# clementabary/music2dance

Hardware: AMD Instinct MI355X
Metric: 120-frame seq/sec, phase3 WGAN-GP step, batch 64 per GPU (higher is better)
Workload: dtype f32

## Files before the change

music2dance_amd/csrc/conv1d_thin.hip:

```cpp
#include "m2d_common.h"

#define THIN_MAX_K 32

struct ThinArgs {
  const float* x;
  const float* w;
  const float* bias;
  const float* dy;
  const float* mask;
  float* out;
  float* out2;
  float* stats;
  int xT, xS, xhop;
  int B, L, Cout, ks, stride, pad, Lout;
  int act;
  float slope, mask_slope;
  int chunk;
};

typedef float thin_f32x16 __attribute__((ext_vector_type(16)));
typedef float thin_f32x4 __attribute__((ext_vector_type(4)));
typedef unsigned thin_u32x4 __attribute__((ext_vector_type(4)));

__device__ __forceinline__ float thin_act(float v, int act, float slope) {
  if (act == 0) return v;
  if (act == 1) return m2d_act_sel(v, 1, 0.f);
  return m2d_act_sel(v, 2, slope);
}

template <int KS, int S, bool MASKED>
__global__ void __launch_bounds__(256) thin_bwd_weight_mfma_kernel(const ThinArgs a) {
  constexpr int LD = 65;
  constexpr int XW = 64 * S + 32;
  constexpr int DEPTH = MASKED ? 1 : 2;
  __shared__ float smem[4][32 * LD + XW];
  const int lane = threadIdx.x & 63, wave = threadIdx.x >> 6;
  const int n = blockIdx.y;
  const int l0 = blockIdx.x * a.chunk;
  int l1 = l0 + a.chunk;
  if (l1 > a.Lout) l1 = a.Lout;
  const float* xr = a.xT > 0 ? a.x + (size_t)(n / a.xT) * a.xS + (size_t)(n % a.xT) * a.xhop : a.x + (size_t)n * a.L;
  const float* dyn = a.dy + (size_t)n * 32 * a.Lout;
  const float* mkn = (MASKED && a.mask) ? a.mask + (size_t)n * 32 * a.Lout : nullptr;
  float* tl = smem[wave];
  float* xw = tl + 32 * LD;
  thin_f32x16 acc;
#pragma unroll
  for (int r = 0; r < 16; ++r) acc[r] = 0.f;
  const int i31 = lane & 31, h = lane >> 5;
  const int lq = 4 * (lane & 15);
  const bool vec = (a.Lout % 4) == 0, vec2 = (a.Lout % 2) == 0 && (l0 & 1) == 0;
  float4 dv[DEPTH][8], mv[MASKED ? 8 : 1];
  float xs[DEPTH][(XW + 63) / 64];
  auto fetch = [&](float4 (&d4)[8], float (&xq)[(XW + 63) / 64], int lt) {
#ifdef THIN_X_BW_NOLOAD
#pragma unroll
    for (int i = 0; i < 8; ++i) {
      d4[i] = make_float4((float)lt, 1.f, 2.f, (float)lane);
      if (MASKED) mv[i] = make_float4(1.f, -1.f, 1.f, (float)(lane - 32));
    }
#pragma unroll
    for (int i = 0; i < (XW + 63) / 64; ++i) xq[i] = (float)(lt + i);
    return;
#endif
#pragma unroll
    for (int i = 0; i < 8; ++i) {
      const int co = (lane >> 4) + 4 * i;
      const size_t g = (size_t)co * a.Lout + lt + lq;
      if (vec && lt + lq + 3 < l1) {
        d4[i] = *reinterpret_cast<const float4*>(dyn + g);
        if (MASKED) mv[i] = mkn ? *reinterpret_cast<const float4*>(mkn + g) : make_float4(1.f, 1.f, 1.f, 1.f);
      } else if (vec2 && lt + lq + 3 < l1) {
        const float2 d0 = *reinterpret_cast<const float2*>(dyn + g);
        const float2 d1 = *reinterpret_cast<const float2*>(dyn + g + 2);
        d4[i] = make_float4(d0.x, d0.y, d1.x, d1.y);
        if (MASKED) {
          if (mkn) {
            const float2 m0 = *reinterpret_cast<const float2*>(mkn + g);
            const float2 m1 = *reinterpret_cast<const float2*>(mkn + g + 2);
            mv[i] = make_float4(m0.x, m0.y, m1.x, m1.y);
          } else {
            mv[i] = make_float4(1.f, 1.f, 1.f, 1.f);
          }
        }
      } else {
        float d[4], m[4];
#pragma unroll
        for (int j = 0; j < 4; ++j) {
          const bool ok = lt + lq + j < l1;
          d[j] = ok ? dyn[g + j] : 0.f;
          m[j] = (MASKED && ok && mkn) ? mkn[g + j] : 1.f;
        }
        d4[i] = make_float4(d[0], d[1], d[2], d[3]);
        if (MASKED) mv[i] = make_float4(m[0], m[1], m[2], m[3]);
      }
    }
#pragma unroll
    for (int i = 0; i < (XW + 63) / 64; ++i) {
      const int e = lane + 64 * i;
      const int pos = lt * S - a.pad + e;
      xq[i] = (e < XW && lt < l1 && pos >= 0 && pos < a.L) ? xr[pos] : 0.f;
    }
  };
  const int lt0 = l0 + wave * 64;
#pragma unroll
  for (int d = 0; d < DEPTH; ++d)
    if (lt0 + 256 * d < l1) fetch(dv[d], xs[d], lt0 + 256 * d);
  for (int lt = lt0; lt < l1; lt += 256) {
#pragma unroll
    for (int i = 0; i < 8; ++i) {
      const int co = (lane >> 4) + 4 * i;
      const float ms = a.mask_slope;
      tl[co * LD + lq + 0] = dv[0][i].x * ((!MASKED || mv[i].x > 0.f) ? 1.f : ms);
      tl[co * LD + lq + 1] = dv[0][i].y * ((!MASKED || mv[i].y > 0.f) ? 1.f : ms);
      tl[co * LD + lq + 2] = dv[0][i].z * ((!MASKED || mv[i].z > 0.f) ? 1.f : ms);
      tl[co * LD + lq + 3] = dv[0][i].w * ((!MASKED || mv[i].w > 0.f) ? 1.f : ms);
    }
#pragma unroll
    for (int i = 0; i < (XW + 63) / 64; ++i)
      if (lane + 64 * i < XW) xw[lane + 64 * i] = xs[0][i];
    __builtin_amdgcn_fence(__ATOMIC_RELEASE, "wavefront");
    __builtin_amdgcn_wave_barrier();
    if (DEPTH == 2) {
#pragma unroll
      for (int i = 0; i < 8; ++i) dv[0][i] = dv[DEPTH - 1][i];
#pragma unroll
      for (int i = 0; i < (XW + 63) / 64; ++i) xs[0][i] = xs[DEPTH - 1][i];
    }
    if (lt + 256 * DEPTH < l1) fetch(dv[DEPTH - 1], xs[DEPTH - 1], lt + 256 * DEPTH);
    const float* xa = xw + S * h + i31;
    const float* bb = tl + i31 * LD + h;
#pragma unroll 8
    for (int j = 0; j < 32; ++j) {
      float av = xa[2 * S * j];
      if (KS < 32) av = i31 == 31 ? 1.f : av;
#ifdef THIN_X_BW_NOMFMA
      acc[j & 15] += av * bb[2 * j];
#else
      acc = __builtin_amdgcn_mfma_f32_32x32x2f32(av, bb[2 * j], acc, 0, 0, 0);
#endif
    }
    __builtin_amdgcn_wave_barrier();
  }
  __syncthreads();
  float* red = &smem[0][0];
#pragma unroll
  for (int r = 0; r < 16; ++r) red[wave * 1024 + ((r & 3) + 8 * (r >> 2) + 4 * h) * 32 + i31] = acc[r];
  __syncthreads();
  const size_t blk = (size_t)blockIdx.y * gridDim.x + blockIdx.x;
  for (int o = threadIdx.x; o < 32 * KS; o += 256) {
    const int co = o / KS, kk = o % KS;
    const int idx = kk * 32 + co;
    a.out[blk * 32 * KS + o] = red[idx] + red[1024 + idx] + red[2048 + idx] + red[3072 + idx];
  }
  if (a.out2 && threadIdx.x < 32) {
    const int idx = 31 * 32 + threadIdx.x;
    a.out2[blk * 32 + threadIdx.x] = red[idx] + red[1024 + idx] + red[2048 + idx] + red[3072 + idx];
  }
}

template <int KS, int S, bool MASKED>
__global__ void __launch_bounds__(256) thin_bwd_data_mfma_kernel(const ThinArgs a) {
  constexpr int LD = 65;
  constexpr int ZLD = 33;
  constexpr int T = (KS + S - 1) / S;
  constexpr int HALO = T - 1;
  constexpr int DEPTH = MASKED ? 1 : 2;
  __shared__ float smem[4][(64 + HALO) * ZLD];
  static_assert((64 + HALO) * ZLD >= 32 * LD, "image size");
  const int lane = threadIdx.x & 63, wave = threadIdx.x >> 6;
  const int l31 = lane & 31, h = lane >> 5;
  const int n = blockIdx.y;
  const int nq = (a.L - 1 + a.pad) / S + 1;
  const int run = a.chunk / 4;
  const int qa = blockIdx.x * a.chunk + wave * run;
  int qb = qa + run;
  if (qb > nq) qb = nq;
  if (qa >= nq) return;
  const float* dyn = a.dy + (size_t)n * 32 * a.Lout;
  const float* mkn = (MASKED && a.mask) ? a.mask + (size_t)n * 32 * a.Lout : nullptr;
  float* dxn = a.out + (size_t)n * a.L;
  float* buf = smem[wave];
  float wa[16];
#pragma unroll
  for (int s2 = 0; s2 < 16; ++s2) wa[s2] = l31 < KS ? a.w[(2 * s2 + h) * KS + l31] : 0.f;
  const int lq = 4 * (lane & 15);
  const bool vec = (a.Lout % 4) == 0, vec2 = (a.Lout % 2) == 0;
  float4 dv[DEPTH][8], mv[MASKED ? 8 : 1];
  auto fetch = [&](float4 (&d4)[8], int lt) {
#pragma unroll
    for (int i = 0; i < 8; ++i) {
      const int co = (lane >> 4) + 4 * i;
      const int l = lt + lq;
      const size_t g = (size_t)co * a.Lout + l;
      if (vec && l >= 0 && l + 3 < a.Lout) {
        d4[i] = *reinterpret_cast<const float4*>(dyn + g);
        if (MASKED) mv[i] = mkn ? *reinterpret_cast<const float4*>(mkn + g) : make_float4(1.f, 1.f, 1.f, 1.f);
      } else if (vec2 && l >= 0 && l + 3 < a.Lout) {
        const float2 d0 = *reinterpret_cast<const float2*>(dyn + g);
        const float2 d1 = *reinterpret_cast<const float2*>(dyn + g + 2);
        d4[i] = make_float4(d0.x, d0.y, d1.x, d1.y);
        if (MASKED) {
          if (mkn) {
            const float2 m0 = *reinterpret_cast<const float2*>(mkn + g);
            const float2 m1 = *reinterpret_cast<const float2*>(mkn + g + 2);
            mv[i] = make_float4(m0.x, m0.y, m1.x, m1.y);
          } else {
            mv[i] = make_float4(1.f, 1.f, 1.f, 1.f);
          }
        }
      } else {
        float d[4], m[4];
#pragma unroll
        for (int j = 0; j < 4; ++j) {
          const bool ok = l + j >= 0 && l + j < a.Lout;
          d[j] = ok ? dyn[(ptrdiff_t)g + j] : 0.f;
          m[j] = (MASKED && ok && mkn) ? mkn[(ptrdiff_t)g + j] : 1.f;
        }
        d4[i] = make_float4(d[0], d[1], d[2], d[3]);
        if (MASKED) mv[i] = make_float4(m[0], m[1], m[2], m[3]);
      }
    }
  };
  auto land = [&](const float4 (&d4)[8]) {
#pragma unroll
    for (int i = 0; i < 8; ++i) {
      const int co = (lane >> 4) + 4 * i;
      const float ms = a.mask_slope;
      buf[co * LD + lq + 0] = d4[i].x * ((!MASKED || mv[i].x > 0.f) ? 1.f : ms);
      buf[co * LD + lq + 1] = d4[i].y * ((!MASKED || mv[i].y > 0.f) ? 1.f : ms);
      buf[co * LD + lq + 2] = d4[i].z * ((!MASKED || mv[i].z > 0.f) ? 1.f : ms);
      buf[co * LD + lq + 3] = d4[i].w * ((!MASKED || mv[i].w > 0.f) ? 1.f : ms);
    }
  };
  auto sync = [&]() {
    __builtin_amdgcn_fence(__ATOMIC_RELEASE, "wavefront");
    __builtin_amdgcn_wave_barrier();
    __builtin_amdgcn_fence(__ATOMIC_ACQUIRE, "wavefront");
  };
  auto zmma = [&](int c0) {
    thin_f32x16 acc;
#pragma unroll
    for (int r = 0; r < 16; ++r) acc[r] = 0.f;
#pragma unroll
    for (int s2 = 0; s2 < 16; ++s2)
      acc = __builtin_amdgcn_mfma_f32_32x32x2f32(wa[s2], buf[(2 * s2 + h) * LD + c0 + l31], acc, 0, 0, 0);
    return acc;
  };
  float carry[3] = {0.f, 0.f, 0.f};
  if (qa > 0) {
    fetch(dv[0], qa - 64);
    land(dv[0]);
    sync();
    const thin_f32x16 z = zmma(32);
    sync();
#pragma unroll
    for (int r = 0; r < 16; ++r)
      if (l31 >= 32 - HALO) buf[(l31 - (32 - HALO)) * ZLD + (r & 3) + 8 * (r >> 2) + 4 * h] = z[r];
    sync();
#pragma unroll
    for (int k = 0; k < 3; ++k) carry[k] = buf[((lane + 64 * k) >> 5) * ZLD + ((lane + 64 * k) & 31)];
    sync();
  }
#pragma unroll
  for (int d = 0; d < DEPTH; ++d)
    if (qa + 64 * d < qb) fetch(dv[d], qa + 64 * d);
  for (int l0 = qa; l0 < qb; l0 += 64) {
    land(dv[0]);
    sync();
    if (DEPTH == 2) {
#pragma unroll
      for (int i = 0; i < 8; ++i) dv[0][i] = dv[1][i];
    }
    if (l0 + 64 * DEPTH < qb) fetch(dv[DEPTH - 1], l0 + 64 * DEPTH);
    const thin_f32x16 z0 = zmma(0), z1 = zmma(32);
    sync();
#pragma unroll
    for (int k = 0; k < 3; ++k) buf[((lane + 64 * k) >> 5) * ZLD + ((lane + 64 * k) & 31)] = carry[k];
#pragma unroll
    for (int r = 0; r < 16; ++r) {
      const int kk = (r & 3) + 8 * (r >> 2) + 4 * h;
      buf[(HALO + l31) * ZLD + kk] = z0[r];
      buf[(HALO + 32 + l31) * ZLD + kk] = z1[r];
    }
    sync();
    float o[S];
#pragma unroll
    for (int rho = 0; rho < S; ++rho) {
      float acc = 0.f;
#pragma unroll
      for (int t = 0; t < T; ++t)
        if (rho + S * t < KS) acc += buf[(HALO + lane - t) * ZLD + rho + S * t];
      o[rho] = acc;
    }
#pragma unroll
    for (int k = 0; k < 3; ++k) carry[k] = buf[(64 + ((lane + 64 * k) >> 5)) * ZLD + ((lane + 64 * k) & 31)];
    sync();
#pragma unroll
    for (int rho = 0; rho < S; ++rho) buf[S * lane + rho] = o[rho];
    sync();
    const int j0 = S * l0 - a.pad;
#pragma unroll
    for (int k = 0; k < S; ++k) {
      const int e = lane + 64 * k;
      const int j = j0 + e;
      if (j >= 0 && j < a.L && l0 + e / S < qb) dxn[j] = buf[e];
    }
    sync();
  }
}

__global__ void __launch_bounds__(256) thin_sum_partials_kernel(const float* partial, float* dw, int nblk, int n_out,
                                                                  const float* partial2, float* out2, int n_out2) {
  __shared__ double part[32][8];
  const int ox = threadIdx.x & 7, g = threadIdx.x >> 3;
  const int nb1 = (n_out + 7) / 8;
  int blk = blockIdx.x;
  if (blk >= nb1) {
    blk -= nb1;
    partial = partial2;
    dw = out2;
    n_out = n_out2;
  }
  const int o = blk * 8 + ox;
  double s = 0.0;
  if (o < n_out)
    for (int b = g; b < nblk; b += 32) s += (double)partial[(size_t)b * n_out + o];
  part[g][ox] = s;
  __syncthreads();
  if (g == 0 && o < n_out) {
    double t = 0.0;
#pragma unroll
    for (int j = 0; j < 32; ++j) t += part[j][ox];
    dw[o] = (float)t;
  }
}

static bool thin_ok(int Cin, int Cout, int ks, int stride) {
  return Cin == 1 && ks == 25 && stride == 4 && Cout == 32;
}

bool m2d_thin_applicable(int Cin, int Cout, int ks, int stride) { return thin_ok(Cin, Cout, ks, stride); }

static int thin_bw_chunk(int B, int Lout) {
  const long long per = ((long long)B * Lout + 511) / 512;
  long long c = (per + 255) / 256 * 256;
  if (c < 1024) c = 1024;
  if (c > 8192) c = 8192;
  return (int)c;
}

size_t m2d_thin_bwd_weight_ws(int B, int Cout, int ks, int Lout) {
  const size_t nblk = (size_t)B * m2d_ceil_div(Lout, thin_bw_chunk(B, Lout));
  return nblk * (Cout * ks + Cout) * sizeof(float);
}

template <int KS, int S>
#ifndef THIN_WPE
#define THIN_WPE 4
#endif
__global__ void __launch_bounds__(256) __attribute__((amdgpu_waves_per_eu(THIN_WPE, 8)))
thin_fwd_mfma_kernel(const ThinArgs a, int tiles_per_row, int total_tiles) {
  constexpr int NS = (KS + 1) / 2;
  constexpr int LDP = 32 + 4;
  __shared__ float img[4][32 * LDP];
  const int lane = threadIdx.x & 63, wave = __builtin_amdgcn_readfirstlane(threadIdx.x >> 6);
  const int c31 = lane & 31, h = lane >> 5;
  float* im = img[wave];
  float wa[NS];
#pragma unroll
  for (int ks = 0; ks < NS; ++ks) {
    const int k = 2 * ks + h;
    wa[ks] = k < KS ? a.w[c31 * KS + k] : 0.f;
  }
  const int nwaves = gridDim.x * 4;
  const int valign = (a.Lout % 4 == 0) ? 4 : (a.Lout % 2 == 0) ? 2 : 1;
  const int cq = lane & 7;
  const int crow = lane >> 3;
  float bv[4];
#pragma unroll
  for (int i = 0; i < 4; ++i) bv[i] = a.bias ? a.bias[crow + 8 * i] : 0.f;
  const float ms = a.mask_slope;
  double st1[4] = {0.0, 0.0, 0.0, 0.0}, st2[4] = {0.0, 0.0, 0.0, 0.0};
  const unsigned row_bytes = (unsigned)a.Lout * 4u;
  const unsigned sample_bytes = 32u * row_bytes;
  constexpr bool LAST_DEAD = (KS & 1) != 0;

  auto fetch = [&](int tile, float (&dst)[NS]) {
    const int n = tile / tiles_per_row;
    const int p0 = (tile - n * tiles_per_row) * 32;
    const float* xr = a.xT > 0 ? a.x + (size_t)(n / a.xT) * a.xS + (size_t)(n % a.xT) * a.xhop : a.x + (size_t)n * a.L;
    const __amdgpu_buffer_rsrc_t rx = __builtin_amdgcn_make_buffer_rsrc((void*)xr, (short)0, (int)((unsigned)a.L * 4u), 0x00020000);
    const int l = p0 + c31;
    const unsigned voff = l < a.Lout ? (unsigned)((l * S - a.pad + h) * 4) : 0x80000000u;
#pragma unroll
    for (int ks = 0; ks < NS; ++ks) {
#ifdef THIN_X_NOGATHER
      dst[ks] = (float)((voff + ks) & 7);
#else
      dst[ks] = __builtin_bit_cast(float, __builtin_amdgcn_raw_buffer_load_b32(rx, (int)voff + 8 * ks, 0, 0));
#endif
    }
    if (LAST_DEAD && h == 1) dst[NS - 1] = 0.f;
  };
  auto process = [&](int tile, const float (&xb)[NS]) {
    const int n = tile / tiles_per_row;
    const int p0 = (tile - n * tiles_per_row) * 32;
    const bool interior = valign == 4 && p0 + 32 <= a.Lout;
    const __amdgpu_buffer_rsrc_t ro = __builtin_amdgcn_make_buffer_rsrc((void*)(a.out + (size_t)n * 32 * a.Lout), (short)0, (int)sample_bytes, 0x00020000);
    const __amdgpu_buffer_rsrc_t rm = __builtin_amdgcn_make_buffer_rsrc((void*)((a.mask ? a.mask : a.out) + (size_t)n * 32 * a.Lout), (short)0,
                                                                        (int)(a.mask ? sample_bytes : 0u), 0x00020000);
    const unsigned eo = (unsigned)crow * row_bytes + (unsigned)(p0 + 4 * cq) * 4u;
    thin_f32x4 mk[4];
    if (interior && a.mask) {
#pragma unroll
      for (int i = 0; i < 4; ++i)
        mk[i] = __builtin_bit_cast(thin_f32x4, __builtin_amdgcn_raw_buffer_load_b128(rm, (int)(eo + (unsigned)(8 * i) * row_bytes), 0, 0));
    }
    thin_f32x16 acc;
#pragma unroll
    for (int r = 0; r < 16; ++r) acc[r] = 0.f;
#pragma unroll
    for (int ks = 0; ks < NS; ++ks) acc = __builtin_amdgcn_mfma_f32_32x32x2f32(wa[ks], xb[ks], acc, 0, 0, 0);
#pragma unroll
    for (int r = 0; r < 16; ++r) im[((r & 3) + 8 * (r >> 2) + 4 * h) * LDP + c31] = acc[r];
    __builtin_amdgcn_fence(__ATOMIC_RELEASE, "wavefront");
    __builtin_amdgcn_wave_barrier();
    __builtin_amdgcn_fence(__ATOMIC_ACQUIRE, "wavefront");
    if (interior) {
#pragma unroll
      for (int i = 0; i < 4; ++i) {
        const int co = crow + 8 * i;
        const thin_f32x4 q = *reinterpret_cast<const thin_f32x4*>(im + co * LDP + 4 * cq);
        thin_f32x4 v;
#pragma unroll
        for (int j = 0; j < 4; ++j) v[j] = thin_act(q[j] + bv[i], a.act, a.slope);
        if (a.mask) {
#pragma unroll
          for (int j = 0; j < 4; ++j) v[j] *= mk[i][j] > 0.f ? 1.f : ms;
        }
#ifdef THIN_X_NOSTORE
        if (v[0] == 12345.678f)
#endif
        __builtin_amdgcn_raw_buffer_store_b128(__builtin_bit_cast(thin_u32x4, v), ro, (int)(eo + (unsigned)(8 * i) * row_bytes), 0, 0);
        st1[i] += (v[0] + v[1]) + (v[2] + v[3]);
        st2[i] += (v[0] * v[0] + v[1] * v[1]) + (v[2] * v[2] + v[3] * v[3]);
      }
    } else {
      const bool whole = p0 + 4 * cq + 4 <= a.Lout;
#pragma unroll 1
      for (int i = 0; i < 4; ++i) {
        const int co = crow + 8 * i;
        const float4 q = *reinterpret_cast<const float4*>(im + co * LDP + 4 * cq);
        const float b_ = i == 0 ? bv[0] : (i == 1 ? bv[1] : (i == 2 ? bv[2] : bv[3]));
        float v[4] = {q.x + b_, q.y + b_, q.z + b_, q.w + b_};
        const size_t o = ((size_t)n * 32 + co) * a.Lout + p0 + 4 * cq;
#pragma unroll
        for (int j = 0; j < 4; ++j) v[j] = thin_act(v[j], a.act, a.slope);
        if (whole && valign == 4) {
          if (a.mask) {
            const float4 m = *reinterpret_cast<const float4*>(a.mask + o);
            v[0] *= m.x > 0.f ? 1.f : ms;
            v[1] *= m.y > 0.f ? 1.f : ms;
            v[2] *= m.z > 0.f ? 1.f : ms;
            v[3] *= m.w > 0.f ? 1.f : ms;
          }
          *reinterpret_cast<float4*>(a.out + o) = make_float4(v[0], v[1], v[2], v[3]);
        } else if (whole && valign == 2) {
          if (a.mask) {
            const float2 m0 = *reinterpret_cast<const float2*>(a.mask + o);
            const float2 m1 = *reinterpret_cast<const float2*>(a.mask + o + 2);
            v[0] *= m0.x > 0.f ? 1.f : ms;
            v[1] *= m0.y > 0.f ? 1.f : ms;
            v[2] *= m1.x > 0.f ? 1.f : ms;
            v[3] *= m1.y > 0.f ? 1.f : ms;
          }
          *reinterpret_cast<float2*>(a.out + o) = make_float2(v[0], v[1]);
          *reinterpret_cast<float2*>(a.out + o + 2) = make_float2(v[2], v[3]);
        } else {
#pragma unroll
          for (int j = 0; j < 4; ++j) {
            if (p0 + 4 * cq + j < a.Lout) {
              float y = v[j];
              if (a.mask) y *= a.mask[o + j] > 0.f ? 1.f : ms;
              a.out[o + j] = y;
              v[j] = y;
            } else {
              v[j] = 0.f;
            }
          }
        }
        {
          const float t1 = (v[0] + v[1]) + (v[2] + v[3]);
          const float t2 = (v[0] * v[0] + v[1] * v[1]) + (v[2] * v[2] + v[3] * v[3]);
          if (i == 0) { st1[0] += t1; st2[0] += t2; }
          else if (i == 1) { st1[1] += t1; st2[1] += t2; }
          else if (i == 2) { st1[2] += t1; st2[2] += t2; }
          else { st1[3] += t1; st2[3] += t2; }
        }
      }
    }
    __builtin_amdgcn_wave_barrier();
  };

  int tile = __builtin_amdgcn_readfirstlane(blockIdx.x * 4 + wave);
  const int gw = tile;
  auto flush_stats = [&]() {
    if (!a.stats) return;
#pragma unroll
    for (int i = 0; i < 4; ++i) {
      double s1 = st1[i], s2 = st2[i];
#pragma unroll
      for (int off = 4; off > 0; off >>= 1) {
        s1 += __shfl_xor(s1, off, 64);
        s2 += __shfl_xor(s2, off, 64);
      }
      if (cq == 0) {
        float* dst = a.stats + (size_t)gw * 64 + 2 * (crow + 8 * i);
        dst[0] = (float)s1;
        dst[1] = (float)s2;
      }
    }
  };
  if (tile >= total_tiles) {
    flush_stats();
    return;
  }
  float xa[NS], xb2[NS];
  fetch(tile, xa);
#pragma unroll 1
  for (;;) {
    const int t2 = tile + nwaves;
    if (t2 < total_tiles) fetch(t2, xb2);
    process(tile, xa);
    if (t2 >= total_tiles) break;
    const int t3 = t2 + nwaves;
    if (t3 < total_tiles) fetch(t3, xa);
    process(t2, xb2);
    if (t3 >= total_tiles) break;
    tile = t3;
  }
  flush_stats();
}

struct M2dWinView {
  int T, S, hop;
};

int m2d_rowsums_reduce(const float* part, int P, int M, double* sums, double* scratch, hipStream_t stream);

static int thin_fwd_tiles_per_row(int Lout) { return m2d_ceil_div(Lout, 32); }
#define THIN_FWD_MAX_WAVES (256 * 16 * 4)
static size_t thin_fwd_stats_part(int B, int Lout) { (void)B; (void)Lout; return (size_t)THIN_FWD_MAX_WAVES * 64 * sizeof(float); }
size_t m2d_thin_fwd_stats_ws(int B, int Lout) { return thin_fwd_stats_part(B, Lout) + (size_t)256 * 32 * 2 * sizeof(double); }
static int thin_fwd_grid(int total_tiles) {
  static const int per_cu = [] { const char* e = getenv("M2D_THIN_WG_PER_CU"); const int v = e ? atoi(e) : THIN_WPE; return v >= 1 && v <= 16 ? v : THIN_WPE; }();
  const int need = m2d_ceil_div(total_tiles, 4), full = 256 * per_cu;
  return need < full ? need : full;
}

int m2d_thin_fwd(const float* x, const float* w, const float* bias, float* y, int B, int L, int Cout, int ks,
                 int stride, int pad, int Lout, int act, float slope, const float* out_mask, float out_mask_slope,
                 const M2dWinView* wv, double* stats, void* ws, size_t ws_bytes, hipStream_t stream) {
  ThinArgs a;
  memset(&a, 0, sizeof(a));
  if (wv) { a.xT = wv->T; a.xS = wv->S; a.xhop = wv->hop; }
  const int tpr = thin_fwd_tiles_per_row(Lout);
  if ((long long)B * tpr >= (1LL << 30) || (long long)Lout * 32 * 4 >= (1LL << 31) || (long long)L * 4 >= (1LL << 31))
    M2D_FAIL(M2D_ERR_RANGE, "m2d_conv1d_fwd (thin): too many tiles / a sample beyond 2 GiB");
  const int total = B * tpr;
  if (stats) {
    if (!ws || ws_bytes < m2d_thin_fwd_stats_ws(B, Lout)) M2D_FAIL(M2D_ERR_WORKSPACE, "m2d_conv1d_fwd (thin): no room for the statistics partials");
    a.stats = (float*)ws;
  }
  a.x = x; a.w = w; a.bias = bias; a.mask = out_mask; a.out = y;
  a.B = B; a.L = L; a.Cout = Cout; a.ks = ks; a.stride = stride; a.pad = pad; a.Lout = Lout;
  a.act = act; a.slope = slope; a.mask_slope = out_mask_slope;
  M2dProfScope prof(M2D_FAM_POINTWISE, stream, 2.0 * B * Lout * (double)Cout * ks,
                    4.0 * B * ((double)L + (double)Cout * Lout * (out_mask ? 2 : 1)), "thin_conv_fwd", Cout, B * Lout, ks);
  const int grid = thin_fwd_grid(total);
  hipLaunchKernelGGL((thin_fwd_mfma_kernel<25, 4>), dim3(grid), dim3(256), 0, stream, a, tpr, total);
  M2D_CHECK_LAUNCH("thin_fwd_mfma_kernel");
  if (stats)
    return m2d_rowsums_reduce(a.stats, grid * 4, 32, stats, (double*)((char*)a.stats + thin_fwd_stats_part(B, Lout)), stream);
  return M2D_OK;
}

template <int KS, int S>
__global__ void __launch_bounds__(512) thin_long_fwd_kernel(const ThinArgs a, int tiles_per_row, int total_tiles) {
  static_assert(KS % 2 == 0 && S % 2 == 0, "even taps / stride");
  constexpr int NS = KS / 2;
  constexpr int SEG = 31 * S + KS + 3;
  constexpr int SEG4 = (SEG + 3) / 4;
  constexpr int NP = (SEG4 + 63) / 64;
  constexpr int LDP = 32 + 4;
  constexpr int WAVE_FLOATS = SEG4 * 4 + 32 * LDP;
  extern __shared__ __attribute__((aligned(16))) float lsm[];
  float* Ws = lsm;
  const int lane = threadIdx.x & 63, wave = __builtin_amdgcn_readfirstlane(threadIdx.x >> 6);
  float* xs = lsm + KS * 32 + wave * WAVE_FLOATS;
  float* im = xs + SEG4 * 4;
  const int c31 = lane & 31, h = lane >> 5;
  const int lead = ((a.pad + 3) & ~3) - a.pad;
  for (int e = threadIdx.x; e < KS * 32; e += 512) {
    const int k = e >> 5, c = e & 31;
    Ws[e] = a.w[c * KS + k];
  }
  __syncthreads();
  const int nwaves = gridDim.x * 8;
  const int cq = lane & 7, crow = lane >> 3;
  float bv[4];
#pragma unroll
  for (int i = 0; i < 4; ++i) bv[i] = a.bias ? a.bias[crow + 8 * i] : 0.f;
  const unsigned row_bytes = (unsigned)a.Lout * 4u;
  const unsigned sample_bytes = 32u * row_bytes;

  thin_f32x4 seg[NP];
  auto fetch = [&](int tile) {
    const int n = tile / tiles_per_row;
    const int p0 = (tile - n * tiles_per_row) * 32;
    const float* xr = a.xT > 0 ? a.x + (size_t)(n / a.xT) * a.xS + (size_t)(n % a.xT) * a.xhop : a.x + (size_t)n * a.L;
    const __amdgpu_buffer_rsrc_t rx = __builtin_amdgcn_make_buffer_rsrc((void*)xr, (short)0, (int)((unsigned)a.L * 4u), 0x00020000);
    const int first = p0 * S - a.pad - lead;
#pragma unroll
    for (int i = 0; i < NP; ++i) {
      const int q = lane + 64 * i;
      const unsigned voff = q < SEG4 ? (unsigned)((first + 4 * q) * 4) : 0x80000000u;
      seg[i] = __builtin_bit_cast(thin_f32x4, __builtin_amdgcn_raw_buffer_load_b128(rx, (int)voff, 0, 0));
    }
  };
  auto land = [&]() {
#pragma unroll
    for (int i = 0; i < NP; ++i) {
      const int q = lane + 64 * i;
      if (q < SEG4) *reinterpret_cast<thin_f32x4*>(xs + 4 * q) = seg[i];
    }
  };
  int tile = __builtin_amdgcn_readfirstlane(blockIdx.x * 8 + wave);
  const int gw = tile;
  double st1[4] = {0.0, 0.0, 0.0, 0.0}, st2[4] = {0.0, 0.0, 0.0, 0.0};
  auto flush_stats = [&]() {
    if (!a.stats) return;
#pragma unroll
    for (int i = 0; i < 4; ++i) {
      double s1 = st1[i], s2 = st2[i];
#pragma unroll
      for (int off = 4; off > 0; off >>= 1) {
        s1 += __shfl_xor(s1, off, 64);
        s2 += __shfl_xor(s2, off, 64);
      }
      if (cq == 0) {
        float* dst = a.stats + (size_t)gw * 64 + 2 * (crow + 8 * i);
        dst[0] = (float)s1;
        dst[1] = (float)s2;
      }
    }
  };
  if (tile >= total_tiles) {
    flush_stats();
    return;
  }
  fetch(tile);
  land();
  __builtin_amdgcn_fence(__ATOMIC_RELEASE, "wavefront");
  __builtin_amdgcn_wave_barrier();
  __builtin_amdgcn_fence(__ATOMIC_ACQUIRE, "wavefront");
  const float* ap = Ws + h * 32 + c31;
  const float* bp = xs + c31 * S + h + lead;
#pragma unroll 1
  for (;;) {
    const int next = tile + nwaves;
    if (next < total_tiles) fetch(next);
    thin_f32x16 acc;
#pragma unroll
    for (int r = 0; r < 16; ++r) acc[r] = 0.f;
#pragma unroll
    for (int ks = 0; ks < NS; ++ks) acc = __builtin_amdgcn_mfma_f32_32x32x2f32(ap[ks * 64], bp[2 * ks], acc, 0, 0, 0);
    const int n = tile / tiles_per_row;
    const int p0 = (tile - n * tiles_per_row) * 32;
#pragma unroll
    for (int r = 0; r < 16; ++r) im[((r & 3) + 8 * (r >> 2) + 4 * h) * LDP + c31] = acc[r];
    __builtin_amdgcn_fence(__ATOMIC_RELEASE, "wavefront");
    __builtin_amdgcn_wave_barrier();
    __builtin_amdgcn_fence(__ATOMIC_ACQUIRE, "wavefront");
    if (next < total_tiles) land();
    const __amdgpu_buffer_rsrc_t ro = __builtin_amdgcn_make_buffer_rsrc((void*)(a.out + (size_t)n * 32 * a.Lout), (short)0, (int)sample_bytes, 0x00020000);
    const unsigned eo = (unsigned)crow * row_bytes + (unsigned)(p0 + 4 * cq) * 4u;
#pragma unroll
    for (int i = 0; i < 4; ++i) {
      const int co = crow + 8 * i;
      const thin_f32x4 q = *reinterpret_cast<const thin_f32x4*>(im + co * LDP + 4 * cq);
      thin_f32x4 v;
#pragma unroll
      for (int j = 0; j < 4; ++j) v[j] = thin_act(q[j] + bv[i], a.act, a.slope);
      __builtin_amdgcn_raw_buffer_store_b128(__builtin_bit_cast(thin_u32x4, v), ro, (int)(eo + (unsigned)(8 * i) * row_bytes), 0, 0);
      st1[i] += (v[0] + v[1]) + (v[2] + v[3]);
      st2[i] += (v[0] * v[0] + v[1] * v[1]) + (v[2] * v[2] + v[3] * v[3]);
    }
    __builtin_amdgcn_fence(__ATOMIC_RELEASE, "wavefront");
    __builtin_amdgcn_wave_barrier();
    __builtin_amdgcn_fence(__ATOMIC_ACQUIRE, "wavefront");
    if (next >= total_tiles) break;
    tile = next;
  }
  flush_stats();
}

static bool thin_long_enabled() {
  static const bool on = [] { const char* e = getenv("M2D_THIN_LONG"); return !(e && e[0] == '0'); }();
  return on;
}
static int thin_long_kind(int Cin, int Cout, int ks, int stride) {
  if (Cin != 1 || Cout != 32) return 0;
  if (ks == 250 && stride == 50) return 1;
  if (ks == 160 && stride == 4) return 2;
  return 0;
}
bool m2d_thin_long_applicable(int Cin, int Cout, int ks, int stride, int pad, int L) {
  if (!thin_long_enabled() || !thin_long_kind(Cin, Cout, ks, stride)) return false;
  if ((L & 3) || pad < 0 || pad >= ks) return false;
  const int Lout = (L + 2 * pad - ks) / stride + 1;
  return Lout > 0 && Lout % 32 == 0;
}
#define THIN_LONG_MAX_WAVES (512 * 8)
size_t m2d_thin_long_stats_ws(int B, int Lout) { (void)B; (void)Lout; return (size_t)THIN_LONG_MAX_WAVES * 64 * sizeof(float) + (size_t)256 * 32 * 2 * sizeof(double); }

template <int KS, int S>
static int thin_long_launch(const ThinArgs& a, int tpr, int total, hipStream_t stream, int* waves) {
  constexpr int SEG4 = (31 * S + KS + 3 + 3) / 4;
  constexpr size_t lds = (size_t)(KS * 32 + 8 * (SEG4 * 4 + 32 * 36)) * sizeof(float);
  static const bool attr_ok = hipFuncSetAttribute(reinterpret_cast<const void*>(&thin_long_fwd_kernel<KS, S>),
                                                  hipFuncAttributeMaxDynamicSharedMemorySize, (int)lds) == hipSuccess;
  if (!attr_ok) M2D_FAIL(M2D_ERR_HIP, "m2d_conv1d_fwd (long single-channel kernel): cannot reserve %zu bytes of LDS", lds);
  const int per_cu = lds * 2 <= 160 * 1024 ? 2 : 1;
  const int need = m2d_ceil_div(total, 8);
  const int grid = need < 256 * per_cu ? need : 256 * per_cu;
  *waves = grid * 8;
  hipLaunchKernelGGL((thin_long_fwd_kernel<KS, S>), dim3(grid), dim3(512), lds, stream, a, tpr, total);
  M2D_CHECK_LAUNCH("thin_long_fwd_kernel");
  return M2D_OK;
}

int m2d_thin_long_fwd(const float* x, const float* w, const float* bias, float* y, int B, int L, int ks, int stride, int pad,
                      int Lout, int act, float slope, const M2dWinView* wv, double* stats, void* ws, size_t ws_bytes,
                      hipStream_t stream) {
  ThinArgs a;
  memset(&a, 0, sizeof(a));
  if (wv) { a.xT = wv->T; a.xS = wv->S; a.xhop = wv->hop; }
  const int tpr = Lout / 32;
  if ((long long)B * tpr >= (1LL << 30) || (long long)Lout * 32 * 4 >= (1LL << 31) || (long long)L * 4 >= (1LL << 31))
    M2D_FAIL(M2D_ERR_RANGE, "m2d_conv1d_fwd (long single-channel kernel): too many tiles / a sample beyond 2 GiB");
  const int total = B * tpr;
  const size_t part = (size_t)THIN_LONG_MAX_WAVES * 64 * sizeof(float);
  if (stats) {
    if (!ws || ws_bytes < m2d_thin_long_stats_ws(B, Lout)) M2D_FAIL(M2D_ERR_WORKSPACE, "m2d_conv1d_fwd (long single-channel kernel): no room for the statistics partials");
    a.stats = (float*)ws;
  }
  a.x = x; a.w = w; a.bias = bias; a.out = y;
  a.B = B; a.L = L; a.Cout = 32; a.ks = ks; a.stride = stride; a.pad = pad; a.Lout = Lout;
  a.act = act; a.slope = slope;
  M2dProfScope prof(M2D_FAM_GEMM, stream, 2.0 * B * Lout * 32.0 * ks, 0.0, "m2d_conv1d_fwd", 32, B * Lout, ks);
  int rc, waves = 0;
  if (thin_long_kind(1, 32, ks, stride) == 1) rc = thin_long_launch<250, 50>(a, tpr, total, stream, &waves);
  else rc = thin_long_launch<160, 4>(a, tpr, total, stream, &waves);
  if (rc) return rc;
  if (stats) return m2d_rowsums_reduce(a.stats, waves, 32, stats, (double*)((char*)a.stats + part), stream);
  return M2D_OK;
}

int m2d_thin_bwd_data(const float* dy, const float* w, float* dx, int B, int L, int Cout, int ks, int stride,
                      int pad, int Lout, const float* dy_mask, float dy_mask_slope, hipStream_t stream) {
  ThinArgs a;
  memset(&a, 0, sizeof(a));
  a.dy = dy; a.w = w; a.mask = dy_mask; a.out = dx;
  a.B = B; a.L = L; a.Cout = Cout; a.ks = ks; a.stride = stride; a.pad = pad; a.Lout = Lout;
  a.mask_slope = dy_mask_slope;
  const int nq = (L - 1 + pad) / stride + 1;
  M2dProfScope prof(M2D_FAM_POINTWISE, stream, 2.0 * B * Lout * (double)Cout * ks,
                    4.0 * B * ((double)L + (double)Cout * Lout * (dy_mask ? 2 : 1)), "thin_conv_bwd_data", 1, B * L, Cout * ks);
  a.chunk = thin_bw_chunk(B, nq);
  const dim3 grid(m2d_ceil_div(nq, a.chunk), B);
  if (dy_mask) hipLaunchKernelGGL((thin_bwd_data_mfma_kernel<25, 4, true>), grid, dim3(256), 0, stream, a);
  else hipLaunchKernelGGL((thin_bwd_data_mfma_kernel<25, 4, false>), grid, dim3(256), 0, stream, a);
  M2D_CHECK_LAUNCH("thin_bwd_data_mfma_kernel");
  return M2D_OK;
}

int m2d_thin_bwd_weight(const float* x, const float* dy, float* dw, float* dbias, int B, int L, int Cout, int ks,
                        int stride, int pad, int Lout, const float* dy_mask, float dy_mask_slope, void* ws,
                        size_t ws_bytes, const M2dWinView* wv, hipStream_t stream) {
  if (!ws || ws_bytes < m2d_thin_bwd_weight_ws(B, Cout, ks, Lout))
    M2D_FAIL(M2D_ERR_WORKSPACE, "m2d_conv1d_bwd_weight (thin): workspace too small");
  ThinArgs a;
  memset(&a, 0, sizeof(a));
  if (wv) { a.xT = wv->T; a.xS = wv->S; a.xhop = wv->hop; }
  a.x = x; a.dy = dy; a.mask = dy_mask; a.out = (float*)ws;
  a.B = B; a.L = L; a.Cout = Cout; a.ks = ks; a.stride = stride; a.pad = pad; a.Lout = Lout;
  a.mask_slope = dy_mask_slope;
  a.chunk = thin_bw_chunk(B, Lout);
  const int nchunk = m2d_ceil_div(Lout, a.chunk);
  M2dProfScope prof(M2D_FAM_POINTWISE, stream, 2.0 * B * Lout * (double)Cout * ks,
                    4.0 * B * ((double)L + (double)Cout * Lout * (dy_mask ? 2 : 1)), "thin_conv_bwd_weight", Cout, ks, B * Lout);
  const size_t nblk = (size_t)nchunk * B;
  a.out2 = dbias ? (float*)ws + nblk * Cout * ks : nullptr;
  if (dy_mask)
    hipLaunchKernelGGL((thin_bwd_weight_mfma_kernel<25, 4, true>), dim3(nchunk, B), dim3(256), 0, stream, a);
  else
    hipLaunchKernelGGL((thin_bwd_weight_mfma_kernel<25, 4, false>), dim3(nchunk, B), dim3(256), 0, stream, a);
  hipLaunchKernelGGL(thin_sum_partials_kernel, dim3(m2d_ceil_div(Cout * ks, 8) + (dbias ? m2d_ceil_div(Cout, 8) : 0)),
                     dim3(256), 0, stream, (const float*)ws, dw, nchunk * B, Cout * ks, (const float*)a.out2, dbias, Cout);
  M2D_CHECK_LAUNCH("thin_bwd_weight_mfma_kernel");
  return M2D_OK;
}
```

Baseline: 5679.

## Add direct buffer-load MFMA kernels for thin conv backward data and weight

Adds new backward-weight and backward-data kernels for the single-input-channel conv (ks=25, stride=4, Cout=32). They read dy directly from global memory into registers with 128-bit buffer loads and feed MFMA from those registers, with loads rotated across multiple register sets to overlap with compute, instead of staging dy tiles through LDS. Out-of-range loads rely on buffer-resource bounds returning zero. The kernels are on by default behind an env switch and guarded by alignment and size checks, at the cost of more register pressure and more complex code.

Result: no change. 5694 (median of 6 runs) (+0.3%).

```diff
diff --git a/music2dance_amd/csrc/conv1d_thin.hip b/music2dance_amd/csrc/conv1d_thin.hip
--- a/music2dance_amd/csrc/conv1d_thin.hip
+++ b/music2dance_amd/csrc/conv1d_thin.hip
@@ -336,6 +336,319 @@
   }
 }
 
+static bool thin_direct_enabled() {
+  static const bool on = [] { const char* e = getenv("M2D_THIN_DIRECT"); return !(e && e[0] == '0'); }();
+  return on;
+}
+
+template <int KS, int S, bool MASKED>
+__global__ void __launch_bounds__(256) thin_bwd_weight_direct_kernel(const ThinArgs a) {
+  constexpr int XW = 64 * S + 32;
+  constexpr int NX = (XW + 63) / 64;
+  __shared__ float smem[4][1024];
+  static_assert(64 * NX <= 1024, "x window");
+  const int lane = threadIdx.x & 63, wave = __builtin_amdgcn_readfirstlane(threadIdx.x >> 6);
+  const int n = blockIdx.y;
+  const int l0 = blockIdx.x * a.chunk;
+  int l1 = l0 + a.chunk;
+  if (l1 > a.Lout) l1 = a.Lout;
+  const float* xr = a.xT > 0 ? a.x + (size_t)(n / a.xT) * a.xS + (size_t)(n % a.xT) * a.xhop : a.x + (size_t)n * a.L;
+  const unsigned sample_bytes = 32u * (unsigned)a.Lout * 4u;
+  const __amdgpu_buffer_rsrc_t rx = __builtin_amdgcn_make_buffer_rsrc((void*)xr, (short)0, (int)((unsigned)a.L * 4u), 0x00020000);
+  const __amdgpu_buffer_rsrc_t rd = __builtin_amdgcn_make_buffer_rsrc((void*)(a.dy + (size_t)n * 32 * a.Lout), (short)0, (int)sample_bytes, 0x00020000);
+  const __amdgpu_buffer_rsrc_t rm = __builtin_amdgcn_make_buffer_rsrc((void*)((MASKED ? a.mask : a.dy) + (size_t)n * 32 * a.Lout), (short)0, (int)sample_bytes, 0x00020000);
+  float* xw = smem[wave];
+  thin_f32x4 acc[2][2];
+#pragma unroll
+  for (int q = 0; q < 4; ++q)
+#pragma unroll
+    for (int r = 0; r < 4; ++r) acc[q >> 1][q & 1][r] = 0.f;
+  const int j15 = lane & 15, k4 = lane >> 4;
+  const int lrow = 4 * k4;
+  const unsigned rowoff = ((unsigned)j15 * (unsigned)a.Lout + (unsigned)lrow) * 4u;
+  const unsigned halfoff = 16u * (unsigned)a.Lout * 4u;
+  auto piece_off = [&](int lt, int p) -> int {
+    const int g = p >> 1, c = p & 1;
+    return lt + 16 * g + lrow < l1 ? (int)(rowoff + (unsigned)c * halfoff + (unsigned)(lt + 16 * g) * 4u) : (int)0x80000000u;
+  };
+  auto load_piece = [&](const __amdgpu_buffer_rsrc_t& r, int off) -> thin_f32x4 {
+    return __builtin_bit_cast(thin_f32x4, __builtin_amdgcn_raw_buffer_load_b128(r, off, 0, 0));
+  };
+  auto fetch_x = [&](float (&xq)[NX], int lt) {
+#pragma unroll
+    for (int i = 0; i < NX; ++i) {
+      const int e = lane + 64 * i;
+      const unsigned voff = (e < XW && lt < l1) ? (unsigned)((lt * S - a.pad + e) * 4) : 0x80000000u;
+      xq[i] = __builtin_bit_cast(float, __builtin_amdgcn_raw_buffer_load_b32(rx, (int)voff, 0, 0));
+    }
+  };
+  auto land_x = [&](const float (&xq)[NX]) {
+#pragma unroll
+    for (int i = 0; i < NX; ++i) xw[lane + 64 * i] = xq[i];
+    __builtin_amdgcn_fence(__ATOMIC_RELEASE, "wavefront");
+    __builtin_amdgcn_wave_barrier();
+  };
+  const float* xa = xw + S * lrow + j15;
+  auto mma_group = [&](const thin_f32x4& b0, const thin_f32x4& b1, int g) {
+#pragma unroll
+    for (int s = 0; s < 4; ++s) {
+      const float a0 = xa[S * (16 * g + s)];
+      float a1 = xa[S * (16 * g + s) + 16];
+      if (KS < 32) a1 = j15 == 15 ? 1.f : a1;
+      acc[0][0] = __builtin_amdgcn_mfma_f32_16x16x4f32(a0, b0[s], acc[0][0], 0, 0, 0);
+      acc[0][1] = __builtin_amdgcn_mfma_f32_16x16x4f32(a0, b1[s], acc[0][1], 0, 0, 0);
+      acc[1][0] = __builtin_amdgcn_mfma_f32_16x16x4f32(a1, b0[s], acc[1][0], 0, 0, 0);
+      acc[1][1] = __builtin_amdgcn_mfma_f32_16x16x4f32(a1, b1[s], acc[1][1], 0, 0, 0);
+    }
+  };
+  const int lt0 = l0 + wave * 64;
+  float xs[NX];
+  if (!MASKED) {
+    thin_f32x4 ta[8], tb[8], tc[8];
+#pragma unroll
+    for (int i = 0; i < 8; ++i) ta[i] = load_piece(rd, piece_off(lt0, i));
+#pragma unroll
+    for (int i = 0; i < 8; ++i) tb[i] = load_piece(rd, piece_off(lt0 + 256, i));
+    fetch_x(xs, lt0);
+#pragma unroll
+    for (int i = 0; i < 8; ++i) tc[i] = load_piece(rd, piece_off(lt0 + 512, i));
+    __builtin_amdgcn_sched_barrier(0);
+    auto step = [&](thin_f32x4 (&t)[8], int lt) {
+      land_x(xs);
+      fetch_x(xs, lt + 256);
+      __builtin_amdgcn_sched_barrier(0);
+#pragma unroll
+      for (int g = 0; g < 4; ++g) {
+        mma_group(t[2 * g], t[2 * g + 1], g);
+        t[2 * g] = load_piece(rd, piece_off(lt + 768, 2 * g));
+        t[2 * g + 1] = load_piece(rd, piece_off(lt + 768, 2 * g + 1));
+        __builtin_amdgcn_sched_barrier(0);
+      }
+      __builtin_amdgcn_wave_barrier();
+    };
+    if (lt0 < l1) {
+      int lt = lt0;
+#pragma unroll 1
+      for (;;) {
+        step(ta, lt);
+        lt += 256;
+        if (lt >= l1) break;
+        step(tb, lt);
+        lt += 256;
+        if (lt >= l1) break;
+        step(tc, lt);
+        lt += 256;
+        if (lt >= l1) break;
+      }
+    }
+  } else {
+    thin_f32x4 d[8], m[8], cur[8];
+    fetch_x(xs, lt0);
+#pragma unroll
+    for (int i = 0; i < 8; ++i) {
+      d[i] = load_piece(rd, piece_off(lt0, i));
+      m[i] = load_piece(rm, piece_off(lt0, i));
+    }
+    const float ms = a.mask_slope;
+#pragma unroll 1
+    for (int lt = lt0; lt < l1; lt += 256) {
+#pragma unroll
+      for (int i = 0; i < 8; ++i) {
+#pragma unroll
+        for (int c = 0; c < 4; ++c) cur[i][c] = d[i][c] * (m[i][c] > 0.f ? 1.f : ms);
+      }
+      land_x(xs);
+      fetch_x(xs, lt + 256);
+#pragma unroll
+      for (int i = 0; i < 8; ++i) {
+        d[i] = load_piece(rd, piece_off(lt + 256, i));
+        m[i] = load_piece(rm, piece_off(lt + 256, i));
+      }
+      __builtin_amdgcn_sched_barrier(0);
+#pragma unroll
+      for (int g = 0; g < 4; ++g) mma_group(cur[2 * g], cur[2 * g + 1], g);
+      __builtin_amdgcn_wave_barrier();
+    }
+  }
+  __syncthreads();
+  float* red = &smem[0][0];
+#pragma unroll
+  for (int q = 0; q < 4; ++q)
+#pragma unroll
+    for (int r = 0; r < 4; ++r) red[wave * 1024 + (16 * (q >> 1) + 4 * k4 + r) * 32 + 16 * (q & 1) + j15] = acc[q >> 1][q & 1][r];
+  __syncthreads();
+  const size_t blk = (size_t)blockIdx.y * gridDim.x + blockIdx.x;
+  for (int o = threadIdx.x; o < 32 * KS; o += 256) {
+    const int co = o / KS, kk = o % KS;
+    const int idx = kk * 32 + co;
+    a.out[blk * 32 * KS + o] = red[idx] + red[1024 + idx] + red[2048 + idx] + red[3072 + idx];
+  }
+  if (a.out2 && threadIdx.x < 32) {
+    const int idx = 31 * 32 + threadIdx.x;
+    a.out2[blk * 32 + threadIdx.x] = red[idx] + red[1024 + idx] + red[2048 + idx] + red[3072 + idx];
+  }
+}
+
+template <int KS, int S, bool MASKED>
+__global__ void __launch_bounds__(256) thin_bwd_data_direct_kernel(const ThinArgs a) {
+  static_assert(S == 4, "a position's S outputs are one 16-byte LDS access");
+  constexpr int ZLD = 36;
+  constexpr int T = (KS + S - 1) / S;
+  constexpr int HALO = T - 1;
+  __shared__ __attribute__((aligned(16))) float smem[4][(64 + HALO) * ZLD];
+  const int lane = threadIdx.x & 63, wave = __builtin_amdgcn_readfirstlane(threadIdx.x >> 6);
+  const int j15 = lane & 15, k4 = lane >> 4;
+  const int n = blockIdx.y;
+  const int nq = (a.L - 1 + a.pad) / S + 1;
+  const int run = a.chunk / 4;
+  const int qa = blockIdx.x * a.chunk + wave * run;
+  int qb = qa + run;
+  if (qb > nq) qb = nq;
+  if (qa >= nq) return;
+  const unsigned sample_bytes = 32u * (unsigned)a.Lout * 4u;
+  const __amdgpu_buffer_rsrc_t rd = __builtin_amdgcn_make_buffer_rsrc((void*)(a.dy + (size_t)n * 32 * a.Lout), (short)0, (int)sample_bytes, 0x00020000);
+  const __amdgpu_buffer_rsrc_t rm = __builtin_amdgcn_make_buffer_rsrc((void*)((MASKED ? a.mask : a.dy) + (size_t)n * 32 * a.Lout), (short)0, (int)sample_bytes, 0x00020000);
+  float* dxn = a.out + (size_t)n * a.L;
+  float* buf = smem[wave];
+  const float ms = a.mask_slope;
+  float wa[2][8];
+#pragma unroll
+  for (int i = 0; i < 8; ++i) {
+    wa[0][i] = a.w[(4 * i + k4) * KS + j15];
+    wa[1][i] = 16 + j15 < KS ? a.w[(4 * i + k4) * KS + 16 + j15] : 0.f;
+  }
+  const unsigned rowoff = ((unsigned)k4 * (unsigned)a.Lout + 4u * (unsigned)j15) * 4u;
+  const unsigned stepoff = 4u * (unsigned)a.Lout * 4u;
+  auto piece_off = [&](int lt, int i) -> int {
+    return (lt < qb && lt + 4 * j15 < a.Lout) ? (int)(rowoff + (unsigned)i * stepoff + (unsigned)lt * 4u) : (int)0x80000000u;
+  };
+  auto load_piece = [&](const __amdgpu_buffer_rsrc_t& r, int off) -> thin_f32x4 {
+    return __builtin_bit_cast(thin_f32x4, __builtin_amdgcn_raw_buffer_load_b128(r, off, 0, 0));
+  };
+  auto sync = [&]() {
+    __builtin_amdgcn_fence(__ATOMIC_RELEASE, "wavefront");
+    __builtin_amdgcn_wave_barrier();
+    __builtin_amdgcn_fence(__ATOMIC_ACQUIRE, "wavefront");
+  };
+  float carry[3] = {0.f, 0.f, 0.f};
+  if (qa > 0) {
+    const int p = qa - 16 + j15;
+    thin_f32x4 z0, z1;
+#pragma unroll
+    for (int r = 0; r < 4; ++r) z0[r] = z1[r] = 0.f;
+    float dq[8];
+#pragma unroll
+    for (int i = 0; i < 8; ++i) {
+      const int off = p < a.Lout ? (int)(((unsigned)(4 * i + k4) * (unsigned)a.Lout + (unsigned)p) * 4u) : (int)0x80000000u;
+      dq[i] = __builtin_bit_cast(float, __builtin_amdgcn_raw_buffer_load_b32(rd, off, 0, 0));
+      if (MASKED) dq[i] *= __builtin_bit_cast(float, __builtin_amdgcn_raw_buffer_load_b32(rm, off, 0, 0)) > 0.f ? 1.f : ms;
+    }
+#pragma unroll
+    for (int i = 0; i < 8; ++i) {
+      z0 = __builtin_amdgcn_mfma_f32_16x16x4f32(wa[0][i], dq[i], z0, 0, 0, 0);
+      z1 = __builtin_amdgcn_mfma_f32_16x16x4f32(wa[1][i], dq[i], z1, 0, 0, 0);
+    }
+    if (j15 >= 16 - HALO) {
+      *reinterpret_cast<thin_f32x4*>(buf + (j15 - (16 - HALO)) * ZLD + 4 * k4) = z0;
+      *reinterpret_cast<thin_f32x4*>(buf + (j15 - (16 - HALO)) * ZLD + 16 + 4 * k4) = z1;
+    }
+    sync();
+#pragma unroll
+    for (int k = 0; k < 3; ++k) carry[k] = buf[((lane + 64 * k) >> 5) * ZLD + ((lane + 64 * k) & 31)];
+    sync();
+  }
+  auto step = [&](thin_f32x4 (&t)[8], int l0, int lnext) {
+    thin_f32x4 acc[2][4];
+#pragma unroll
+    for (int q = 0; q < 8; ++q)
+#pragma unroll
+      for (int r = 0; r < 4; ++r) acc[q >> 2][q & 3][r] = 0.f;
+#pragma unroll
+    for (int i = 0; i < 8; ++i) {
+#pragma unroll
+      for (int e = 0; e < 4; ++e) {
+        acc[0][e] = __builtin_amdgcn_mfma_f32_16x16x4f32(wa[0][i], t[i][e], acc[0][e], 0, 0, 0);
+        acc[1][e] = __builtin_amdgcn_mfma_f32_16x16x4f32(wa[1][i], t[i][e], acc[1][e], 0, 0, 0);
+      }
+      if (!MASKED) {
+        t[i] = load_piece(rd, piece_off(lnext, i));
+        __builtin_amdgcn_sched_barrier(0);
+      }
+    }
+#pragma unroll
+    for (int k = 0; k < 3; ++k) buf[((lane + 64 * k) >> 5) * ZLD + ((lane + 64 * k) & 31)] = carry[k];
+#pragma unroll
+    for (int e = 0; e < 4; ++e) {
+      *reinterpret_cast<thin_f32x4*>(buf + (HALO + 4 * j15 + e) * ZLD + 4 * k4) = acc[0][e];
+      *reinterpret_cast<thin_f32x4*>(buf + (HALO + 4 * j15 + e) * ZLD + 16 + 4 * k4) = acc[1][e];
+    }
+    sync();
+    thin_f32x4 o;
+#pragma unroll
+    for (int rho = 0; rho < S; ++rho) o[rho] = 0.f;
+#pragma unroll
+    for (int tt = 0; tt < T; ++tt) {
+      const thin_f32x4 v = *reinterpret_cast<const thin_f32x4*>(buf + (HALO + lane - tt) * ZLD + S * tt);
+#pragma unroll
+      for (int rho = 0; rho < S; ++rho)
+        if (rho + S * tt < KS) o[rho] += v[rho];
+    }
+#pragma unroll
+    for (int k = 0; k < 3; ++k) carry[k] = buf[(64 + ((lane + 64 * k) >> 5)) * ZLD + ((lane + 64 * k) & 31)];
+    sync();
+    *reinterpret_cast<thin_f32x4*>(buf + S * lane) = o;
+    sync();
+    const int j0 = S * l0 - a.pad;
+#pragma unroll
+    for (int k = 0; k < S; ++k) {
+      const int e = lane + 64 * k;
+      const int j = j0 + e;
+      if (j >= 0 && j < a.L && l0 + e / S < qb) dxn[j] = buf[e];
+    }
+    sync();
+  };
+  if (!MASKED) {
+    thin_f32x4 ta[8], tb[8];
+#pragma unroll
+    for (int i = 0; i < 8; ++i) ta[i] = load_piece(rd, piece_off(qa, i));
+#pragma unroll
+    for (int i = 0; i < 8; ++i) tb[i] = load_piece(rd, piece_off(qa + 64, i));
+    __builtin_amdgcn_sched_barrier(0);
+    int l0 = qa;
+#pragma unroll 1
+    for (;;) {
+      step(ta, l0, l0 + 128);
+      l0 += 64;
+      if (l0 >= qb) break;
+      step(tb, l0, l0 + 128);
+      l0 += 64;
+      if (l0 >= qb) break;
+    }
+  } else {
+    thin_f32x4 d[8], m[8], cur[8];
+#pragma unroll
+    for (int i = 0; i < 8; ++i) {
+      d[i] = load_piece(rd, piece_off(qa, i));
+      m[i] = load_piece(rm, piece_off(qa, i));
+    }
+#pragma unroll 1
+    for (int l0 = qa; l0 < qb; l0 += 64) {
+#pragma unroll
+      for (int i = 0; i < 8; ++i) {
+#pragma unroll
+        for (int c = 0; c < 4; ++c) cur[i][c] = d[i][c] * (m[i][c] > 0.f ? 1.f : ms);
+      }
+#pragma unroll
+      for (int i = 0; i < 8; ++i) {
+        d[i] = load_piece(rd, piece_off(l0 + 64, i));
+        m[i] = load_piece(rm, piece_off(l0 + 64, i));
+      }
+      __builtin_amdgcn_sched_barrier(0);
+      step(cur, l0, 0);
+    }
+  }
+}
+
 static bool thin_ok(int Cin, int Cout, int ks, int stride) {
   return Cin == 1 && ks == 25 && stride == 4 && Cout == 32;
 }
@@ -780,7 +1093,10 @@
                     4.0 * B * ((double)L + (double)Cout * Lout * (dy_mask ? 2 : 1)), "thin_conv_bwd_data", 1, B * L, Cout * ks);
   a.chunk = thin_bw_chunk(B, nq);
   const dim3 grid(m2d_ceil_div(nq, a.chunk), B);
-  if (dy_mask) hipLaunchKernelGGL((thin_bwd_data_mfma_kernel<25, 4, true>), grid, dim3(256), 0, stream, a);
+  const bool direct = thin_direct_enabled() && Lout % 4 == 0 && (long long)Lout * 32 * 4 < (1LL << 31);
+  if (direct && dy_mask) hipLaunchKernelGGL((thin_bwd_data_direct_kernel<25, 4, true>), grid, dim3(256), 0, stream, a);
+  else if (direct) hipLaunchKernelGGL((thin_bwd_data_direct_kernel<25, 4, false>), grid, dim3(256), 0, stream, a);
+  else if (dy_mask) hipLaunchKernelGGL((thin_bwd_data_mfma_kernel<25, 4, true>), grid, dim3(256), 0, stream, a);
   else hipLaunchKernelGGL((thin_bwd_data_mfma_kernel<25, 4, false>), grid, dim3(256), 0, stream, a);
   M2D_CHECK_LAUNCH("thin_bwd_data_mfma_kernel");
   return M2D_OK;
@@ -803,7 +1119,13 @@
                     4.0 * B * ((double)L + (double)Cout * Lout * (dy_mask ? 2 : 1)), "thin_conv_bwd_weight", Cout, ks, B * Lout);
   const size_t nblk = (size_t)nchunk * B;
   a.out2 = dbias ? (float*)ws + nblk * Cout * ks : nullptr;
-  if (dy_mask)
+  const bool direct = thin_direct_enabled() && Lout % 4 == 0 && a.chunk % 4 == 0 && (long long)Lout * 32 * 4 < (1LL << 31) &&
+                      (long long)L * 4 < (1LL << 31);
+  if (direct && dy_mask)
+    hipLaunchKernelGGL((thin_bwd_weight_direct_kernel<25, 4, true>), dim3(nchunk, B), dim3(256), 0, stream, a);
+  else if (direct)
+    hipLaunchKernelGGL((thin_bwd_weight_direct_kernel<25, 4, false>), dim3(nchunk, B), dim3(256), 0, stream, a);
+  else if (dy_mask)
     hipLaunchKernelGGL((thin_bwd_weight_mfma_kernel<25, 4, true>), dim3(nchunk, B), dim3(256), 0, stream, a);
   else
     hipLaunchKernelGGL((thin_bwd_weight_mfma_kernel<25, 4, false>), dim3(nchunk, B), dim3(256), 0, stream, a);
```
